# Alanlee0323/ISWM

Measured on AMD Instinct MI355X. Metric: training images/sec (513x513) DeepLabV3+-ResNet101, higher is better.
Workload: dtype f32; 1 GPU; deeplabv3plus_resnet101 output_stride=16, 513x513 synthetic tiles, 16 images/GPU (BASELINE.json configs[2]: global batch 128 over 8 GPUs), weighted CE [1,3], SGD-nesterov + cosine LR; fp32 tensors, conv products via six bf16 MFMAs on an exact 3-way operand split (bf16x6, fp32-level error); conv_math=bf16x6, global_batch=16, parallelism=dp1

## Files before the change

### include/iswm_hip.h

```cpp
#ifndef ISWM_HIP_H
#define ISWM_HIP_H

#include <stddef.h>
#include <stdint.h>

#ifdef __cplusplus
extern "C" {
#endif

typedef void* iswm_stream_t;

const char* iswm_last_error(void);
int iswm_version(void);

typedef struct {
    int N, H, W, Cin;
    int Ho, Wo, Cout;
    int KH, KW, stride, pad, dil;
    int ldx;
    int ldy;
} iswm_conv_desc;

int iswm_set_conv_math(int mode);
int iswm_get_conv_math(void);
// ... 73 lines not shown
int iswm_conv2d_wgrad_planes(const iswm_conv_desc* d, const void* xp, int64_t x_ps, const void* dyp, int64_t dy_ps, float* dw,
                             float* workspace, size_t workspace_bytes, iswm_stream_t stream);
int iswm_dwconv2d_fwd(const iswm_conv_desc* d, const float* x, const float* w, int Cw, const float* bias, float* y,
                      iswm_stream_t stream);
int iswm_dwconv2d_dgrad(const iswm_conv_desc* d, const float* dy, const float* w, int Cw, float* dx, int accumulate,
                        iswm_stream_t stream);
size_t iswm_dwconv2d_wgrad_workspace(const iswm_conv_desc* d);
int iswm_dwconv2d_wgrad(const iswm_conv_desc* d, const float* x, const float* dy, int Cw, float* dw, void* workspace,
                        size_t workspace_bytes, iswm_stream_t stream);
size_t iswm_conv2d_wgrad_workspace(const iswm_conv_desc* d);
int iswm_conv2d_wgrad(const iswm_conv_desc* d, const float* x, const float* dy, float* dw,
                      float* workspace, size_t workspace_bytes, iswm_stream_t stream);

int iswm_colstat_tiles(int64_t M);
int64_t iswm_colstat_tile_rows(int64_t M);
int iswm_colstat(const float* x, int64_t M, int C, int ld, float* partials, iswm_stream_t stream);
int iswm_bn_finalize(const float* partials, int tiles, int C, int64_t count, int64_t tile_rows,
                     const float* gamma, const float* beta, float* running_mean, float* running_var, float momentum,
                     float eps, float* scale, float* shift, float* save_mean, float* save_invstd,
                     iswm_stream_t stream);
int iswm_bn_eval_coeffs(int C, const float* gamma, const float* beta, const float* running_mean,
                        const float* running_var, float eps, float* scale, float* shift,
                        float* save_mean, float* save_invstd, iswm_stream_t stream);
int iswm_bn_apply(const float* y, int64_t M, int C, int ldy, const float* scale, const float* shift,
                  const float* mean, const float* residual, int ldr, int relu, float* out, int ldo,
                  iswm_stream_t stream);
size_t iswm_bn_bwd_workspace(int64_t M, int C);
int iswm_bn_backward(const float* dout, int ldd, const float* out, int ldo, const float* y, int ldy,
                     int64_t M, int C, const float* mean, const float* invstd, const float* gamma,
                     const float* mask_scale, const float* mask_shift,
                     int relu, int training, float* dgamma, float* dbeta, float* dy, int lddy,
                     float* dres, int lddres, void* workspace, size_t workspace_bytes,
                     iswm_stream_t stream);
int iswm_colsum_finalize(const float* partials, int tiles, int C, float* out, float* scratch,
                         iswm_stream_t stream);

int iswm_maxpool3x3s2_fwd(const float* x, int N, int H, int W, int C, float* y, uint8_t* idx, int Ho,
                          int Wo, iswm_stream_t stream);
int iswm_maxpool3x3s2_bwd(const float* dy, const uint8_t* idx, int N, int H, int W, int C, int Ho,
                          int Wo, float* dx, iswm_stream_t stream);
int iswm_gap_fwd(const float* x, int N, int HW, int C, int ldx, float* y, iswm_stream_t stream);
int iswm_gap_bwd(const float* dy, int N, int HW, int C, float* dx, int lddx, int accumulate,
                 iswm_stream_t stream);
int iswm_bcast_fwd(const float* v, int N, int HW, int C, float* y, int ldy, iswm_stream_t stream);
int iswm_bcast_bwd(const float* dy, int lddy, int N, int HW, int C, float* dv, iswm_stream_t stream);

int iswm_bilinear_fwd(const float* x, int N, int Hi, int Wi, int C, int ldx, float* y, int Ho, int Wo,
                      int ldy, iswm_stream_t stream);
int iswm_bilinear_bwd(const float* dy, int N, int Hi, int Wi, int C, int lddy, int Ho, int Wo, float* dx,
                      int lddx, iswm_stream_t stream);
int iswm_bilinear_nhwc_to_nchw_fwd(const float* x, int N, int Hi, int Wi, int C, int ldx, float* y,
                                   int Ho, int Wo, iswm_stream_t stream);
int iswm_bilinear_nhwc_to_nchw_bwd(const float* dy, int N, int Hi, int Wi, int C, int lddx, int Ho,
                                   int Wo, float* dx, iswm_stream_t stream);

int iswm_nchw_to_nhwc(const float* x, int N, int C, int HW, float* y, int Cp, iswm_stream_t stream);
int iswm_nhwc_to_nchw(const float* x, int N, int C, int HW, int ldx, float* y, iswm_stream_t stream);
int iswm_copy_channels(const float* src, int lds, float* dst, int ldd, int64_t M, int C,
                       iswm_stream_t stream);
int iswm_add_inplace(float* dst, const float* src, int64_t n, iswm_stream_t stream);
int iswm_scale_inplace(float* x, int64_t n, const float* scalar_dev, float host_mul, iswm_stream_t stream);
int iswm_bn_apply_classify(const float* y, int64_t M, int C, int ldy, const float* scale, const float* shift, const float* mean,
                           const float* wc4, const float* bias4, float* logits, int ldl, iswm_stream_t stream);
size_t iswm_bn_classify_bwd_workspace(int64_t M, int C);
int iswm_bn_backward_classify(const float* dlogit, int ldl, const float* wc4, const float* y, int ldy, int64_t M, int C,
                              const float* mean, const float* invstd, const float* gamma, const float* mask_scale,
// ... 118 lines not shown
```

### iswm_amd/_lib.py

```python
import ctypes
import os
from ctypes import POINTER, Structure, c_char_p, c_double, c_float, c_int, c_int64, c_size_t, c_uint64, c_void_p

HERE = os.path.dirname(os.path.abspath(__file__))
LIB_PATH = os.path.join(HERE, "libiswm_hip.so")


class ConvDesc(Structure):
    _fields_ = [(n, c_int) for n in ("N", "H", "W", "Cin", "Ho", "Wo", "Cout", "KH", "KW", "stride", "pad",
                                     "dil", "ldx", "ldy")]


class QConvDesc(Structure):
    _fields_ = [(n, c_int) for n in ("N", "H", "W", "Cin", "Ho", "Wo", "Cout", "KH", "KW", "stride", "pad",
                                     "dil", "ldx", "ldy", "ldr", "relu", "lo", "out_f32", "cstore")]


P = c_void_p
_SIGS = {
    "iswm_last_error": (c_char_p, []),
    "iswm_version": (c_int, []),
    "iswm_set_conv_math": (c_int, [c_int]),
    "iswm_get_conv_math": (c_int, []),
    "iswm_conv2d_kernel_name": (c_int, [POINTER(ConvDesc), c_int, c_char_p, c_int]),
# ... 20 lines not shown
    "iswm_maxpool3x3s2_fwd_pl": (c_int, [P, c_int, c_int, c_int, c_int, P, c_int64, P, c_int, c_int, P]),
    "iswm_gap_fwd_pl": (c_int, [P, c_int64, c_int, c_int, c_int, c_int, P, P]),
    "iswm_bcast_fwd_pl": (c_int, [P, c_int, c_int, c_int, P, c_int, c_int64, P]),
    "iswm_bilinear_fwd_pl": (c_int, [P, c_int, c_int, c_int, c_int, c_int, P, c_int64, c_int, c_int, c_int, P]),
    "iswm_conv2d_pl2_weight_bytes": (c_size_t, [POINTER(ConvDesc), c_int]),
    "iswm_conv2d_pl2_pack_weights": (c_int, [POINTER(ConvDesc), c_int, P, P, P]),
    "iswm_conv2d_pl2_tile_rows": (c_int, [POINTER(ConvDesc), c_int]),
    "iswm_conv2d_fwd_pl2": (c_int, [POINTER(ConvDesc), P, c_int64, P, P, P, P, P]),
    "iswm_conv2d_dgrad_pl2": (c_int, [POINTER(ConvDesc), P, c_int64, P, P, c_int, P]),
    "iswm_conv2d_dgrad_pl2_stat_tiles": (c_int, [POINTER(ConvDesc)]),
    "iswm_conv2d_dgrad_pl2_bn": (c_int, [POINTER(ConvDesc), P, c_int64, P, P, c_int, P, c_int, P, P, P, P, c_int, P, c_int, P,
                                         c_int, P]),
    "iswm_bn_backward_stats_pl": (c_int, [P, c_int, P, c_int, c_int64, P, c_int, c_int64, c_int, P, P, P, P, P, c_int, c_int, P, P,
                                          P, c_int, c_int64, P, c_int, P, c_int, P, c_size_t, P]),
    "iswm_aspp_plan_bytes": (c_size_t, [POINTER(ConvDesc), c_int, POINTER(c_int), POINTER(c_int), c_int]),
    "iswm_aspp_plan": (c_int, [POINTER(ConvDesc), c_int, POINTER(c_int), POINTER(c_int), c_int, P, c_int]),
    "iswm_aspp_fwd": (c_int, [POINTER(ConvDesc), c_int, POINTER(c_int), POINTER(c_int), P, P, c_int64, POINTER(c_void_p),
                              POINTER(c_void_p), POINTER(c_void_p), P]),
    "iswm_aspp_bwd": (c_int, [POINTER(ConvDesc), c_int, POINTER(c_int), POINTER(c_int), P, P, c_int64, c_int, POINTER(c_void_p), P,
                              c_int, P, c_int64, POINTER(c_void_p), P, c_size_t, P]),
    "iswm_conv2d_wgrad_planes_ok": (c_int, [POINTER(ConvDesc)]),
    "iswm_conv2d_wgrad_planes_workspace": (c_size_t, [POINTER(ConvDesc)]),
    "iswm_conv2d_wgrad_planes": (c_int, [POINTER(ConvDesc), P, c_int64, P, c_int64, P, P, c_size_t, P]),
    "iswm_conv2d_wgrad_workspace": (c_size_t, [POINTER(ConvDesc)]),
    "iswm_dwconv2d_fwd": (c_int, [POINTER(ConvDesc), P, P, c_int, P, P, P]),
    "iswm_dwconv2d_dgrad": (c_int, [POINTER(ConvDesc), P, P, c_int, P, c_int, P]),
    "iswm_dwconv2d_wgrad_workspace": (c_size_t, [POINTER(ConvDesc)]),
    "iswm_dwconv2d_wgrad": (c_int, [POINTER(ConvDesc), P, P, c_int, P, P, c_size_t, P]),
    "iswm_conv2d_wgrad": (c_int, [POINTER(ConvDesc), P, P, P, P, c_size_t, P]),
    "iswm_colstat_tiles": (c_int, [c_int64]),
    "iswm_colstat_tile_rows": (c_int64, [c_int64]),
    "iswm_colstat": (c_int, [P, c_int64, c_int, c_int, P, P]),
    "iswm_bn_finalize": (c_int, [P, c_int, c_int, c_int64, c_int64, P, P, P, P, c_float, c_float, P, P, P, P, P]),
    "iswm_bn_eval_coeffs": (c_int, [c_int, P, P, P, P, c_float, P, P, P, P, P]),
    "iswm_bn_apply": (c_int, [P, c_int64, c_int, c_int, P, P, P, P, c_int, c_int, P, c_int, P]),
    "iswm_bn_bwd_workspace": (c_size_t, [c_int64, c_int]),
    "iswm_bn_backward": (c_int, [P, c_int, P, c_int, P, c_int, c_int64, c_int, P, P, P, P, P, c_int, c_int, P, P, P, c_int,
                                 P, c_int, P, c_size_t, P]),
    "iswm_colsum_finalize": (c_int, [P, c_int, c_int, P, P, P]),
    "iswm_maxpool3x3s2_fwd": (c_int, [P, c_int, c_int, c_int, c_int, P, P, c_int, c_int, P]),
    "iswm_maxpool3x3s2_bwd": (c_int, [P, P, c_int, c_int, c_int, c_int, c_int, c_int, P, P]),
    "iswm_gap_fwd": (c_int, [P, c_int, c_int, c_int, c_int, P, P]),
    "iswm_gap_bwd": (c_int, [P, c_int, c_int, c_int, P, c_int, c_int, P]),
    "iswm_bcast_fwd": (c_int, [P, c_int, c_int, c_int, P, c_int, P]),
    "iswm_bcast_bwd": (c_int, [P, c_int, c_int, c_int, c_int, P, P]),
    "iswm_bilinear_fwd": (c_int, [P, c_int, c_int, c_int, c_int, c_int, P, c_int, c_int, c_int, P]),
    "iswm_bilinear_bwd": (c_int, [P, c_int, c_int, c_int, c_int, c_int, c_int, c_int, P, c_int, P]),
    "iswm_bilinear_nhwc_to_nchw_fwd": (c_int, [P, c_int, c_int, c_int, c_int, c_int, P, c_int, c_int, P]),
    "iswm_bilinear_nhwc_to_nchw_bwd": (c_int, [P, c_int, c_int, c_int, c_int, c_int, c_int, c_int, P, P]),
    "iswm_nchw_to_nhwc": (c_int, [P, c_int, c_int, c_int, P, c_int, P]),
    "iswm_nhwc_to_nchw": (c_int, [P, c_int, c_int, c_int, c_int, P, P]),
    "iswm_copy_channels": (c_int, [P, c_int, P, c_int, c_int64, c_int, P]),
    "iswm_add_inplace": (c_int, [P, P, c_int64, P]),
    "iswm_scale_inplace": (c_int, [P, c_int64, P, c_float, P]),
    "iswm_bn_apply_classify": (c_int, [P, c_int64, c_int, c_int, P, P, P, P, P, P, c_int, P]),
    "iswm_bn_classify_bwd_workspace": (c_size_t, [c_int64, c_int]),
    "iswm_bn_backward_classify": (c_int, [P, c_int, P, P, c_int, c_int64, c_int, P, P, P, P, P, c_int, P, P, P, P, c_int, c_int64,
                                          P, c_size_t, P]),
    "iswm_pad_weights": (c_int, [P, c_int, c_int, c_int, c_int, P, c_int, c_int, P, P]),
    "iswm_unpad_weights": (c_int, [P, c_int, c_int, c_int, c_int, c_int, c_int, P, P, P]),
    "iswm_fill_zero": (c_int, [P, c_size_t, P]),
    "iswm_zero_cols": (c_int, [P, c_int64, c_int64, c_int, c_int, c_int64, c_int, P]),
    "iswm_dropout_fwd": (c_int, [P, P, P, c_int64, c_float, c_uint64, c_uint64, P]),
    "iswm_dropout_bwd": (c_int, [P, P, P, c_int64, c_float, P]),
    "iswm_loss_blocks": (c_int, [c_int64]),
    "iswm_loss_fwd": (c_int, [P, P, c_int, c_int, c_int, c_int64, P, c_int, c_float, c_float, c_int, P, P, P]),
# ... 71 lines not shown
```

### iswm_amd/csrc/bn.hip

```cpp
#include <stdlib.h>

#include "rowmap.h"

namespace iswm {

__global__ __launch_bounds__(256) void k_colstat(const float* __restrict__ x, int64_t M, int C4, int ld,
                                                 int CQ, int RL, int tiles, int C, int64_t R,
                                                 float* __restrict__ partials) {
    __shared__ float red[256 * 4];
    __shared__ float mean_s[256 * 4];
    RowThread rt = row_thread(C4, CQ, RL);
    const int t = threadIdx.x;
    const int64_t r_begin = (int64_t)blockIdx.x * R;
    const int64_t r_end = min(M, r_begin + R);
    const float cnt = (float)(r_end - r_begin);
    const float* p = x + rt.c4 * 4;
    float4 s = make_float4(0, 0, 0, 0);
    if (rt.active)
        for (int64_t r = r_begin + rt.rl; r < r_end; r += RL) {
            float4 v = ld4(p + r * ld);
            s.x += v.x; s.y += v.y; s.z += v.z; s.w += v.w;
        }
    st4(&red[t * 4], s);
    __syncthreads();
// ... 350 lines not shown
    }
    for (int64_t r = rt.row0; r < M; r += rt.rstep) {
        float4 g = ld4(dout + r * ldd + c);
        float4 v = make_float4(0.f, 0.f, 0.f, 0.f);
        if (TRAIN || RELU == 2) v = ld4(y + r * ldy + c);
        if (RELU == 1) {
            float4 o = ld4x_hi(out, r * ldo + c, ops);
            g.x = o.x > 0.f ? g.x : 0.f; g.y = o.y > 0.f ? g.y : 0.f;
            g.z = o.z > 0.f ? g.z : 0.f; g.w = o.w > 0.f ? g.w : 0.f;
        } else if (RELU == 3) {
            float4 o = ld4x_hi(out, r * ldo + c, ops);
            g.x = (o.x > 0.f && o.x < 6.f) ? g.x : 0.f; g.y = (o.y > 0.f && o.y < 6.f) ? g.y : 0.f;
            g.z = (o.z > 0.f && o.z < 6.f) ? g.z : 0.f; g.w = (o.w > 0.f && o.w < 6.f) ? g.w : 0.f;
        } else if (RELU == 2) {
            g.x = (v.x - mu.x) * msc.x + msh.x > 0.f ? g.x : 0.f;
            g.y = (v.y - mu.y) * msc.y + msh.y > 0.f ? g.y : 0.f;
            g.z = (v.z - mu.z) * msc.z + msh.z > 0.f ? g.z : 0.f;
            g.w = (v.w - mu.w) * msc.w + msh.w > 0.f ? g.w : 0.f;
        }
        if (DRES) st4(dres + r * lddres + c, g);
        const double gd[4] = {g.x, g.y, g.z, g.w};
        float d[4];
        if (TRAIN) {
            const double vd[4] = {v.x, v.y, v.z, v.w};
#pragma unroll
            for (int k = 0; k < 4; ++k)
                d[k] = (float)(gi[k] * (gd[k] - k1[k] - (vd[k] - mud[k]) * isd[k] * k2[k]));
        } else {
#pragma unroll
            for (int k = 0; k < 4; ++k) d[k] = (float)(gi[k] * gd[k]);
        }
        st4x(dy, r * lddy + c, dyps, make_float4(d[0], d[1], d[2], d[3]));
    }
}

static int chk_rows(const char* what, int64_t M, int C, int ld) {
    ISWM_REQUIRE(M > 0 && C > 0 && C % 4 == 0 && ld % 4 == 0 && ld >= C, "%s: bad shape M=%lld C=%d ld=%d", what,
                 (long long)M, C, ld);
    return 0;
}

}

using namespace iswm;

extern "C" int iswm_colstat_tiles(int64_t M) {
    int64_t t = (M + 31) / 32;
    if (t > 1024) t = 1024;
    if (t < 1) t = 1;
    return (int)t;
}

extern "C" int64_t iswm_colstat_tile_rows(int64_t M) {
    const int64_t tiles = iswm_colstat_tiles(M);
    return (M + tiles - 1) / tiles;
}

extern "C" int iswm_colstat(const float* x, int64_t M, int C, int ld, float* partials, iswm_stream_t stream) {
    if (int e = chk_rows("colstat", M, C, ld)) return e;
    ISWM_REQUIRE(x && partials && aligned16(x) && aligned16(partials), "colstat: bad pointer");
    const int64_t R = iswm_colstat_tile_rows(M);
    const int tiles = (int)((M + R - 1) / R);
    RowPlan p = plan_rows(M, C, tiles);
    hipLaunchKernelGGL(k_colstat, dim3(p.rowblocks, p.colblocks), dim3(256), 0, (hipStream_t)stream, x, M, p.C4,
                       ld, p.CQ, p.RL, tiles, C, R, partials);
    return check_launch("colstat");
// ... 56 lines not shown
    hipStream_t s = (hipStream_t)stream;
    if (out_ps != 0 && C % 8 == 0 && ldy % 8 == 0 && ldo % 8 == 0 && aligned16(out) && (out_ps < 0 || out_ps % 8 == 0) &&
        (!residual || (ldr % 8 == 0 && aligned16(residual) && (res_ps <= 0 || res_ps % 8 == 0)))) {
        RowPlan p = plan_rows(M, C / 2);
        dim3 grid(p.rowblocks, p.colblocks), blk(256);
#define LAUNCH8(R, S) \
    hipLaunchKernelGGL((k_bn_apply8<R, S>), grid, blk, 0, s, y, M, p.C4, ldy, scale, shift, mean, residual, ldr, rps, out, \
                       ldo, ops, p.CQ, p.RL)
        ISWM_REQUIRE(relu == 0 || relu == 1 || relu == 6, "bn_apply: relu must be 0 (none), 1 (ReLU) or 6 (ReLU6)");
        if (relu == 6 && residual) LAUNCH8(2, true);
        else if (relu == 6) LAUNCH8(2, false);
        else if (relu && residual) LAUNCH8(1, true);
        else if (relu) LAUNCH8(1, false);
        else if (residual) LAUNCH8(0, true);
        else LAUNCH8(0, false);
#undef LAUNCH8
        return check_launch("bn_apply8");
    }
    RowPlan p = plan_rows(M, C);
    dim3 grid(p.rowblocks, p.colblocks), blk(256);
#define LAUNCH(R, S) \
    hipLaunchKernelGGL((k_bn_apply<R, S>), grid, blk, 0, s, y, M, p.C4, ldy, scale, shift, mean, residual, ldr, rps, out, \
                       ldo, ops, \
                       p.CQ, p.RL)
    ISWM_REQUIRE(relu == 0 || relu == 1 || relu == 6, "bn_apply: relu must be 0 (none), 1 (ReLU) or 6 (ReLU6)");
    if (relu == 6 && residual) LAUNCH(2, true);
    else if (relu == 6) LAUNCH(2, false);
    else if (relu && residual) LAUNCH(1, true);
    else if (relu) LAUNCH(1, false);
    else if (residual) LAUNCH(0, true);
    else LAUNCH(0, false);
#undef LAUNCH
    return check_launch("bn_apply");
}

extern "C" size_t iswm_bn_bwd_workspace(int64_t M, int C) {
    return ((size_t)2 * iswm_colstat_tiles(M) * C + (size_t)2 * C) * sizeof(double);
}

extern "C" int iswm_bn_backward(const float* dout, int ldd, const float* out, int ldo, const float* y, int ldy,
                                int64_t M, int C, const float* mean, const float* invstd, const float* gamma,
                                const float* mask_scale, const float* mask_shift,
                                int relu, int training, float* dgamma, float* dbeta, float* dy, int lddy,
                                float* dres, int lddres, void* workspace, size_t workspace_bytes,
                                iswm_stream_t stream) {
    return iswm_bn_backward_pl(dout, ldd, out, ldo, 0, y, ldy, M, C, mean, invstd, gamma, mask_scale, mask_shift, relu,
                               training, dgamma, dbeta, dy, lddy, 0, dres, lddres, workspace, workspace_bytes, stream);
}

static int bn_backward_impl(const float* dout, int ldd, const void* out, int ldo, int64_t out_ps, const float* y,
                            int ldy, int64_t M, int C, const float* mean, const float* invstd, const float* gamma,
                            const float* mask_scale, const float* mask_shift, int relu, int training,
                            float* dgamma, float* dbeta, void* dy, int lddy, int64_t dy_ps, float* dres,
                            int lddres, void* workspace, size_t workspace_bytes, const double* ready_partials,
                            int ready_tiles, iswm_stream_t stream) {
    if (int e = chk_rows("bn_backward", M, C, ldy)) return e;
    if (int e = chk_ps("bn_backward(dy)", dy, M, lddy, dy_ps)) return e;
    if (out) if (int e = chk_ps("bn_backward(out)", out, M, ldo, out_ps)) return e;
    const int64_t ops = out_ps, dyps = dy_ps;
    ISWM_REQUIRE(relu == 0 || relu == 1 || relu == 6, "bn_backward: relu must be 0 (none), 1 (ReLU) or 6 (ReLU6)");
    const bool relu6 = relu == 6;
    const bool masky = relu == 1 && !dres && mask_scale && mask_shift;
    ISWM_REQUIRE(dout && y && mean && invstd && dgamma && dbeta && dy && workspace && (!relu || out || masky),
                 "bn_backward: null pointer");
    ISWM_REQUIRE(ldd % 4 == 0 && ldd >= C && lddy % 4 == 0 && lddy >= C && (!relu || (ldo % 4 == 0 && ldo >= C)) &&
                     (!dres || (lddres % 4 == 0 && lddres >= C)),
                 "bn_backward: bad pitch");
    ISWM_REQUIRE(workspace_bytes >= iswm_bn_bwd_workspace(M, C) && aligned16(workspace),
                 "bn_backward: workspace too small");
    const int tiles = ready_partials ? ready_tiles : iswm_colstat_tiles(M);
    const double* partials = ready_partials ? ready_partials : (const double*)workspace;
    double* sums = (double*)workspace + (size_t)2 * iswm_colstat_tiles(M) * C;
    hipStream_t s = (hipStream_t)stream;
    if (!ready_partials) {
        double* partials = (double*)workspace;
        RowPlan p = plan_rows(M, C, tiles);
        dim3 grid(p.rowblocks, p.colblocks), blk(256);
#define RLAUNCH(R, D)                                                                                           \
    hipLaunchKernelGGL((k_bn_bwd_reduce<R, D>), grid, blk, 0, s, dout, ldd, out, ldo, ops, y, ldy, M, p.C4, C, mean, invstd, \
                       mask_scale, mask_shift, p.CQ, p.RL, tiles, partials)
        const bool dbl = M <= 8192;
        if (relu6 && dbl) RLAUNCH(3, true);
        else if (relu6) RLAUNCH(3, false);
        else if (masky && dbl) RLAUNCH(2, true);
        else if (masky) RLAUNCH(2, false);
        else if (relu && dbl) RLAUNCH(1, true);
        else if (relu) RLAUNCH(1, false);
        else if (dbl) RLAUNCH(0, true);
        else RLAUNCH(0, false);
#undef RLAUNCH
        if (int e = check_launch("bn_bwd_reduce")) return e;
    }
    if (tiles > 32)
        hipLaunchKernelGGL((k_bn_bwd_finalize<double, 4>), dim3((C + 3) / 4), dim3(256), 0, s, partials, tiles, C,
                           dgamma, dbeta, sums);
    else
        hipLaunchKernelGGL((k_bn_bwd_finalize<double, 16>), dim3((C + 15) / 16), dim3(256), 0, s, partials, tiles, C,
                           dgamma, dbeta, sums);
    if (int e = check_launch("bn_bwd_finalize")) return e;
    const double inv = 1.0 / (double)M;
    RowPlan p = plan_rows(M, C);
    dim3 grid(p.rowblocks, p.colblocks), blk(256);
#define LAUNCH(R, T, D)                                                                                          \
    hipLaunchKernelGGL((k_bn_bwd_apply<R, T, D>), grid, blk, 0, s, dout, ldd, out, ldo, ops, y, ldy, M, p.C4, C, mean,    \
                       invstd, gamma, mask_scale, mask_shift, sums, inv, dy, lddy, dyps, dres, lddres, p.CQ, p.RL)
    const int key = (relu ? 4 : 0) | (training ? 2 : 0) | (dres ? 1 : 0);
    if (relu6) {
        if (training && dres) LAUNCH(3, true, true);
        else if (training) LAUNCH(3, true, false);
        else if (dres) LAUNCH(3, false, true);
        else LAUNCH(3, false, false);
    } else if (masky) {
        if (training) LAUNCH(2, true, false);
        else LAUNCH(2, false, false);
    } else switch (key) {
        case 0: LAUNCH(0, false, false); break;
        case 1: LAUNCH(0, false, true); break;
        case 2: LAUNCH(0, true, false); break;
        case 3: LAUNCH(0, true, true); break;
        case 4: LAUNCH(1, false, false); break;
        case 5: LAUNCH(1, false, true); break;
        case 6: LAUNCH(1, true, false); break;
        default: LAUNCH(1, true, true); break;
    }
#undef LAUNCH
// ... 34 lines not shown
```

### iswm_amd/network/_hip.py

```python

import torch
import torch.nn as nn

from .. import ops


MASK_RECORDER = None
POOL_RECORDER = None
CALIB_RECORDER = None


def pad4(c):
    return (c + 3) // 4 * 4


def pad_cin(c):
    if c % 32 == 0 or c < 128:
        return pad4(c)
    return (c + 31) // 32 * 32


def dense_flat(t):
    if t.dim() == 4 and not t.is_contiguous():
        v = t.permute(0, 2, 3, 1)
# ... 250 lines not shown
    sep = None
    if isinstance(conv, SeparableBase):
        sep, conv = conv, conv.body[1]
        x = sep.body[0].fwd(x, save)
    training = bn.training
    if bn.momentum is None or not bn.track_running_stats or not bn.affine:
        raise NotImplementedError("HIP BatchNorm2d supports affine=True, momentum!=None, running stats")
    if isinstance(conv, DepthwiseConv2d):
        g = conv.geometry(x)
        y = conv.fwd(x, save)
        partials, tiles = None, (0, 0)
        if training:
            partials, nt, tr = ops.colstat(y)
            tiles = (nt, tr)
        return _cba_finish(conv, bn, relu, x, y, g, partials, tiles, training, save, residual, out, sep, True, out_fmt)
    g = conv.geometry(x)
    if conv.bias is None:
        y, partials, tiles = ops.conv2d_fwd(x, conv.ohwi(), g, want_stats=training, wpk=conv.packed(0), wpk2=conv.packed2(0))
    else:
        y, _, _ = ops.conv2d_fwd(x, conv.ohwi(), g, bias=conv.bias_p())
        partials, tiles = None, (0, 0)
        if training:
            partials, nt, tr = ops.colstat(y)
            tiles = (nt, tr)
    return _cba_finish(conv, bn, relu, x, y, g, partials, tiles, training, save, residual, out, sep, False, out_fmt)


def _cba_finish(conv, bn, relu, x, y, g, partials, tiles, training, save, residual, out, sep, dw, out_fmt=None):
    if training:
        count = y.shape[0] * y.shape[1] * y.shape[2]
        if count <= 1:
            raise ValueError("Expected more than 1 value per channel when training, got input size %s" %
                             (tuple(y.shape),))
        coef = ops.bn_finalize(partials, tiles[0], count, tiles[1], bn.weight, bn.bias, bn.running_mean, bn.running_var,
                               bn.momentum, bn.eps)
        if not getattr(bn, "_iswm_nbt_fused", False):
            bn.num_batches_tracked.add_(1)
    else:
        coef = ops.bn_eval_coeffs(bn.weight, bn.bias, bn.running_mean, bn.running_var, bn.eps)
    if out_fmt is None:
        want_planes = ops.planes_on() and y.shape[3] % 64 == 0
    else:
        want_planes = out_fmt == "planes" and ops.planes_on() and y.shape[3] % 64 == 0
    o = ops.bn_apply(y, coef, relu, residual, out, planes=want_planes)
    if MASK_RECORDER is not None and relu:
        of = ops.as_f32(o)
        MASK_RECORDER[bn] = (of > 0) & (of < 6) if relu == 6 and relu is not True else (of > 0)
    if CALIB_RECORDER is not None:
        CALIB_RECORDER.record(conv, o)
    ctx = None
    if save:
        ctx = dict(x=x, y=y, out=o, coef=coef, g=g, relu=relu, training=training, res=residual is not None, sep=sep, dw=dw)
    return o, ctx


_BN3_FUSE = True


def _bn_stats_request(up):
    if up is None or not ops.planes_on() or up.get("bn_stats") is not None:
        return None
    if ops._relu_code(up["relu"]) not in (0, 1):
        return None
    if up.get("res"):
        if not (_BN3_FUSE and ops._relu_code(up["relu"]) == 1 and ops.is_planes(up["out"]) and up["training"]):
            return None
        return ops.BnStats(up["y"], up["coef"], up["relu"], mask=up["out"])
    return ops.BnStats(up["y"], up["coef"], up["relu"])


def cba_bwd_bn(conv, bn, ctx, dout, sink, dy_out=None, need_dx=True):
    y, o = ctx["y"], ctx["out"]
    sep = ctx.get("sep")
    if sep is not None:
        conv = sep.body[1]
    gw, gb = bn.weight, bn.bias
    dgamma = sink.target(gw) if gw.requires_grad else torch.empty_like(gw)
# ... 271 lines not shown
```

### iswm_amd/ops.py

```python
import ctypes
import functools

import torch

from . import _lib
from ._lib import ConvDesc, call

BN_EPS = 1e-5


def _stream():
    return ctypes.c_void_p(torch.cuda.current_stream().cuda_stream)


def _p(t):
    return ctypes.c_void_p(t.data_ptr()) if t is not None else None


def geom(t, dtype=torch.float32):
    if isinstance(t, Planes):
        raise ValueError("this operation takes an fp32 NHWC tensor, not Planes (use .f32())")
    if t.dim() != 4 or t.dtype != dtype or not t.is_cuda:
        raise ValueError("expected a 4-D fp32 CUDA NHWC tensor, got %s %s %s" % (tuple(t.shape), t.dtype, t.device))
    n, h, w, c = t.shape
# ... 600 lines not shown
    coef = torch.empty((4, c), dtype=torch.float32, device=partials.device)
    call("iswm_bn_finalize", _p(partials), tiles, c, count, tile_rows, _p(gamma), _p(beta), _p(running_mean),
         _p(running_var), float(momentum), float(eps), _p(coef[0]), _p(coef[1]), _p(coef[2]), _p(coef[3]), _stream())
    return coef


def bn_eval_coeffs(gamma, beta, running_mean, running_var, eps=BN_EPS):
    c = running_mean.numel()
    coef = torch.empty((4, c), dtype=torch.float32, device=running_mean.device)
    call("iswm_bn_eval_coeffs", c, _p(gamma), _p(beta), _p(running_mean), _p(running_var), float(eps), _p(coef[0]),
         _p(coef[1]), _p(coef[2]), _p(coef[3]), _stream())
    return coef


def _relu_code(relu):
    return 6 if (relu == 6 and relu is not True) else int(bool(relu))


def bn_apply(y, coef, relu, residual=None, out=None, planes=False):
    m, c, ldy = rows(y)
    if out is None:
        out = new_planes(*y.shape, y.device) if planes else torch.empty(y.shape, dtype=torch.float32, device=y.device)
    po, mo, co, ldo, pso = xrows(out)
    assert (mo, co) == (m, c)
    pr, ldr, psr = None, 0, 0
    if residual is not None:
        pr, mr, cr, ldr, psr = xrows(residual)
        assert (mr, cr) == (m, c)
    call("iswm_bn_apply_pl", _p(y), m, c, ldy, _p(coef[0]), _p(coef[1]), _p(coef[2]), _p(pr), ldr, psr, _relu_code(relu),
         _p(po), ldo, pso, _stream())
    return out


def bn_backward(dout, out, y, coef, gamma, relu, training, dgamma, dbeta, want_dres=False, dy=None, dy_planes=False,
                stats=None):
    m, c, ldy = rows(y)
    _, _, ldd = rows(dout)
    po, ldo, pso = None, 0, 0
    if out is not None:
        po, _, _, ldo, pso = xrows(out)
    need = _lib.load().iswm_bn_bwd_workspace(m, c)
    ws = torch.empty((need // 8,), dtype=torch.float64, device=y.device)
    if dy is None:
        dy = new_planes(*y.shape, y.device) if dy_planes else torch.empty(y.shape, dtype=torch.float32, device=y.device)
    pdy, _, _, lddy, psdy = xrows(dy)
    dres = torch.empty(y.shape, dtype=torch.float32, device=y.device) if want_dres else None
    masky = _relu_code(relu) == 1 and not want_dres
    if stats is not None and stats.partials is not None:
        call("iswm_bn_backward_stats_pl", _p(dout), ldd, _p(po), ldo, pso, _p(y), ldy, m, c, _p(coef[2]), _p(coef[3]), _p(gamma),
             _p(coef[0]) if masky else None, _p(coef[1]) if masky else None,
             _relu_code(relu), int(bool(training)), _p(dgamma), _p(dbeta), _p(pdy), lddy, psdy, _p(dres),
             rows(dres)[2] if dres is not None else 0, _p(stats.partials), stats.tiles, _p(ws), need, _stream())
        return dy, dres
    call("iswm_bn_backward_pl", _p(dout), ldd, _p(po), ldo, pso, _p(y), ldy, m, c, _p(coef[2]), _p(coef[3]), _p(gamma),
         _p(coef[0]) if masky else None, _p(coef[1]) if masky else None,
         _relu_code(relu), int(bool(training)), _p(dgamma), _p(dbeta), _p(pdy), lddy, psdy, _p(dres),
         rows(dres)[2] if dres is not None else 0, _p(ws), need, _stream())
    return dy, dres


def bn_apply_classify(y, coef, wc4, bias4):
    m, c, ldy = rows(y)
    out = torch.empty(tuple(y.shape[:3]) + (4,), dtype=torch.float32, device=y.device)
    call("iswm_bn_apply_classify", _p(y), m, c, ldy, _p(coef[0]), _p(coef[1]), _p(coef[2]), _p(wc4), _p(bias4), _p(out), 4, _stream())
    return out

# ... 465 lines not shown
```

Measured before the change: 268.1 images/sec.

## Fold BN statistic finalization into the apply and backward-apply kernels

Adds fused kernels that reduce the per-tile BN partial sums to mean/variance (or dgamma/dbeta) inside each block and then apply the normalization or backward input-gradient in the same launch. This removes a separate finalize launch and its global round-trip for the coefficients, in both forward and backward training paths. Each block redundantly re-reduces the partials for its channel group, adding duplicated reduction work and shared-memory use. The fused path applies only when tiles is between 33 and 128 and C is a multiple of 32; otherwise it falls back to the old two-step path.

```diff
diff --git a/include/iswm_hip.h b/include/iswm_hip.h
--- a/include/iswm_hip.h
+++ b/include/iswm_hip.h
@@ -129,6 +129,13 @@
                      int relu, int training, float* dgamma, float* dbeta, float* dy, int lddy,
                      float* dres, int lddres, void* workspace, size_t workspace_bytes,
                      iswm_stream_t stream);
+int iswm_bn_finalize_apply_pl(const float* partials, int tiles, int C, int64_t count, int64_t tile_rows,
+                              const float* gamma, const float* beta, float* running_mean, float* running_var,
+                              float momentum, float eps, float* scale, float* shift, float* save_mean,
+                              float* save_invstd, const float* y, int64_t M, int ldy, const void* residual, int ldr,
+                              int64_t res_ps, int relu, void* out, int ldo, int64_t out_ps, iswm_stream_t stream);
+int iswm_bn_set_fold(int on);
+int iswm_bn_fold_applies(int tiles, int C);
 int iswm_colsum_finalize(const float* partials, int tiles, int C, float* out, float* scratch,
                          iswm_stream_t stream);
 
diff --git a/iswm_amd/_lib.py b/iswm_amd/_lib.py
--- a/iswm_amd/_lib.py
+++ b/iswm_amd/_lib.py
@@ -76,6 +76,10 @@
     "iswm_colstat_tile_rows": (c_int64, [c_int64]),
     "iswm_colstat": (c_int, [P, c_int64, c_int, c_int, P, P]),
     "iswm_bn_finalize": (c_int, [P, c_int, c_int, c_int64, c_int64, P, P, P, P, c_float, c_float, P, P, P, P, P]),
+    "iswm_bn_finalize_apply_pl": (c_int, [P, c_int, c_int, c_int64, c_int64, P, P, P, P, c_float, c_float, P, P, P, P,
+                                          P, c_int64, c_int, P, c_int, c_int64, c_int, P, c_int, c_int64, P]),
+    "iswm_bn_set_fold": (c_int, [c_int]),
+    "iswm_bn_fold_applies": (c_int, [c_int, c_int]),
     "iswm_bn_eval_coeffs": (c_int, [c_int, P, P, P, P, c_float, P, P, P, P, P]),
     "iswm_bn_apply": (c_int, [P, c_int64, c_int, c_int, P, P, P, P, c_int, c_int, P, c_int, P]),
     "iswm_bn_bwd_workspace": (c_size_t, [c_int64, c_int]),
diff --git a/iswm_amd/csrc/bn.hip b/iswm_amd/csrc/bn.hip
--- a/iswm_amd/csrc/bn.hip
+++ b/iswm_amd/csrc/bn.hip
@@ -406,6 +406,283 @@
         }
         st4x(dy, r * lddy + c, dyps, make_float4(d[0], d[1], d[2], d[3]));
     }
+}
+
+constexpr int FOLD_G = 32;
+constexpr int FOLD_TL = 64;
+constexpr int FOLD_LPT = FOLD_TL * FOLD_G / 256;
+constexpr int FOLD_MAX_TILES = 2 * FOLD_TL;
+
+template <int RELU, bool RES, bool W8>
+__global__ __launch_bounds__(256) void k_bn_fin_apply(const float* __restrict__ partials, int tiles, int C, double count,
+                                                      double R, const float* __restrict__ gamma,
+                                                      const float* __restrict__ beta, float* running_mean,
+                                                      float* running_var, float momentum, float eps, float* scale,
+                                                      float* shift, float* save_mean, float* save_invstd,
+                                                      const float* __restrict__ y, int64_t M, int ldy,
+                                                      const void* __restrict__ res, int ldr, int64_t rps,
+                                                      void* __restrict__ out, int ldo, int64_t ops) {
+    constexpr int NU = W8 ? 2 : 1;
+    constexpr int TPR = FOLD_G / (4 * NU);
+    constexpr int RLN = 256 / TPR;
+    __shared__ double red[FOLD_TL][FOLD_G];
+    __shared__ double mean_s[FOLD_G];
+    __shared__ __align__(16) float coef_s[3][FOLD_G];
+    __shared__ double nt_s[FOLD_MAX_TILES];
+    const int t = threadIdx.x;
+    const int c0 = blockIdx.y * FOLD_G;
+    const int cq = (t % TPR) * 4 * NU;
+    const int c = c0 + cq;
+    int64_t r = (int64_t)blockIdx.x * RLN + t / TPR;
+    const int64_t rstep = (int64_t)gridDim.x * RLN;
+    const float4 z4 = make_float4(0.f, 0.f, 0.f, 0.f);
+    float4 v[2][NU], q[2][NU];
+    auto load = [&](int64_t r0) {
+#pragma unroll
+        for (int u = 0; u < 2; ++u) {
+            const int64_t rr = r0 + u * rstep;
+#pragma unroll
+            for (int n = 0; n < NU; ++n) v[u][n] = q[u][n] = z4;
+            if (rr < M) {
+#pragma unroll
+                for (int n = 0; n < NU; ++n) v[u][n] = ld4(y + rr * ldy + c + 4 * n);
+                if (RES) {
+                    if constexpr (W8) ld8x(res, rr * ldr + c, rps, q[u][0], q[u][1]);
+                    else q[u][0] = ld4x(res, rr * ldr + c, rps);
+                }
+            }
+        }
+    };
+    load(r);
+
+    const int cl = t % FOLD_G, j = t / FOLD_G;
+    const int pc = c0 + cl;
+    float sv[FOLD_LPT][2], qv[FOLD_LPT][2];
+    const float* ps = partials + c0;
+    const float* pq = ps + (size_t)tiles * C;
+#pragma unroll
+    for (int i = 0; i < FOLD_LPT; ++i)
+#pragma unroll
+        for (int h = 0; h < 2; ++h) {
+            const int k = j + FOLD_LPT * i + FOLD_TL * h;
+            const unsigned off = (unsigned)(min(k, tiles - 1) * C + cl);
+            sv[i][h] = ps[off];
+            qv[i][h] = pq[off];
+        }
+#pragma unroll
+    for (int i = 0; i < FOLD_LPT; ++i)
+#pragma unroll
+        for (int h = 0; h < 2; ++h)
+            if (j + FOLD_LPT * i + FOLD_TL * h >= tiles) sv[i][h] = qv[i][h] = 0.f;
+    if (t < tiles) nt_s[t] = R > 0.0 ? fmin(R, count - (double)t * R) : (double)partials[(size_t)2 * tiles * C + t];
+#pragma unroll
+    for (int i = 0; i < FOLD_LPT; ++i) {
+        double s = 0.0;
+        s += (double)sv[i][0];
+        s += (double)sv[i][1];
+        red[j + FOLD_LPT * i][cl] = s;
+    }
+    __syncthreads();
+    if (t < FOLD_G) {
+        double s = red[0][cl];
+#pragma unroll 9
+        for (int k = 1; k < FOLD_TL; ++k) s += red[k][cl];
+        mean_s[cl] = s / count;
+    }
+    __syncthreads();
+    const double mean = mean_s[cl];
+#pragma unroll
+    for (int i = 0; i < FOLD_LPT; ++i) {
+        double m2 = 0.0;
+#pragma unroll
+        for (int h = 0; h < 2; ++h) {
+            const int k = j + FOLD_LPT * i + FOLD_TL * h;
+            if (k < tiles) {
+                const double nt = nt_s[k];
+                const double d = (double)sv[i][h] / nt - mean;
+                m2 += (double)qv[i][h] + nt * d * d;
+            }
+        }
+        red[j + FOLD_LPT * i][cl] = m2;
+        __builtin_amdgcn_sched_barrier(0);
+    }
+    __syncthreads();
+    if (t < FOLD_G) {
+        double m2 = red[0][cl];
+#pragma unroll 9
+        for (int k = 1; k < FOLD_TL; ++k) m2 += red[k][cl];
+        double var = m2 / count;
+        if (var < 0.0) var = 0.0;
+        float invstd = (float)(1.0 / sqrt(var + (double)eps));
+        float g = gamma ? gamma[pc] : 1.f, b = beta ? beta[pc] : 0.f;
+        float sc = g * invstd;
+        coef_s[0][cl] = sc;
+        coef_s[1][cl] = b;
+        coef_s[2][cl] = (float)mean;
+        if (blockIdx.x == 0) {
+            scale[pc] = sc;
+            shift[pc] = b;
+            save_mean[pc] = (float)mean;
+            save_invstd[pc] = invstd;
+            if (running_mean) {
+                double unbiased = count > 1.0 ? var * count / (count - 1.0) : var;
+                running_mean[pc] = __fadd_rn(__fmul_rn(1.f - momentum, running_mean[pc]), __fmul_rn(momentum, (float)mean));
+                running_var[pc] = __fmaf_rn(momentum, (float)unbiased, __fmul_rn(1.f - momentum, running_var[pc]));
+            }
+        }
+    }
+    __syncthreads();
+    float4 sc[NU], sh[NU], mu[NU];
+#pragma unroll
+    for (int n = 0; n < NU; ++n) {
+        sc[n] = ld4(&coef_s[0][cq + 4 * n]);
+        sh[n] = ld4(&coef_s[1][cq + 4 * n]);
+        mu[n] = ld4(&coef_s[2][cq + 4 * n]);
+    }
+    auto one = [&](int64_t rr, const float4* vv, const float4* qq) {
+        float4 o[NU];
+#pragma unroll
+        for (int n = 0; n < NU; ++n) {
+            o[n].x = (vv[n].x - mu[n].x) * sc[n].x + sh[n].x; o[n].y = (vv[n].y - mu[n].y) * sc[n].y + sh[n].y;
+            o[n].z = (vv[n].z - mu[n].z) * sc[n].z + sh[n].z; o[n].w = (vv[n].w - mu[n].w) * sc[n].w + sh[n].w;
+            if (RES) {
+                o[n].x += qq[n].x; o[n].y += qq[n].y; o[n].z += qq[n].z; o[n].w += qq[n].w;
+            }
+            if (RELU) {
+                o[n].x = fmaxf(o[n].x, 0.f); o[n].y = fmaxf(o[n].y, 0.f); o[n].z = fmaxf(o[n].z, 0.f); o[n].w = fmaxf(o[n].w, 0.f);
+            }
+            if (RELU == 2) {
+                o[n].x = fminf(o[n].x, 6.f); o[n].y = fminf(o[n].y, 6.f); o[n].z = fminf(o[n].z, 6.f); o[n].w = fminf(o[n].w, 6.f);
+            }
+        }
+        if constexpr (W8) st8x(out, rr * ldo + c, ops, o[0], o[1]);
+        else st4x(out, rr * ldo + c, ops, o[0]);
+    };
+    while (r < M) {
+        one(r, v[0], q[0]);
+        if (r + rstep < M) one(r + rstep, v[1], q[1]);
+        r += 2 * rstep;
+        if (r < M) load(r);
+    }
+}
+
+template <int RELU, bool DRES>
+__global__ __launch_bounds__(256, 5) void k_bn_bwd_fin_apply(const float* __restrict__ dout, int ldd,
+                                                          const void* __restrict__ out, int ldo, int64_t ops,
+                                                          const float* __restrict__ y, int ldy, int64_t M, int C,
+                                                          const float* __restrict__ mean, const float* __restrict__ invstd,
+                                                          const float* __restrict__ gamma, const float* __restrict__ mscale,
+                                                          const float* __restrict__ mshift,
+                                                          const double* __restrict__ partials, int tiles, double inv_count,
+                                                          float* dgamma, float* dbeta, void* __restrict__ dy, int lddy,
+                                                          int64_t dyps, float* __restrict__ dres, int lddres) {
+    constexpr int TPR = FOLD_G / 4, RLN = 256 / TPR;
+    __shared__ double red[FOLD_TL][FOLD_G];
+    __shared__ double sum_s[2][FOLD_G];
+    const int t = threadIdx.x;
+    const int c0 = blockIdx.y * FOLD_G;
+    const int cq = (t % TPR) * 4;
+    const int c = c0 + cq;
+    int64_t r = (int64_t)blockIdx.x * RLN + t / TPR;
+    const int64_t rstep = (int64_t)gridDim.x * RLN;
+    const float4 z4 = make_float4(0.f, 0.f, 0.f, 0.f);
+    float4 g = z4, v = z4, o = z4;
+    auto load_o = [&](int64_t rr) {
+        if (RELU == 1 || RELU == 3) o = ld4x_hi(out, rr * ldo + c, ops);
+    };
+    auto load = [&](int64_t rr) {
+        g = ld4(dout + rr * ldd + c);
+        v = ld4(y + rr * ldy + c);
+    };
+    if (r < M) load(r);
+
+    const int cl = t % FOLD_G, j = t / FOLD_G;
+    const int pc = c0 + cl;
+#pragma unroll
+    for (int w = 0; w < 2; ++w) {
+        const double* pw = partials + (size_t)w * tiles * C + c0;
+        double a[FOLD_LPT][2];
+#pragma unroll
+        for (int i = 0; i < FOLD_LPT; ++i)
+#pragma unroll
+            for (int h = 0; h < 2; ++h) {
+                const int k = j + FOLD_LPT * i + FOLD_TL * h;
+                a[i][h] = pw[(unsigned)(min(k, tiles - 1) * C + cl)];
+            }
+        if (w) __syncthreads();
+#pragma unroll
+        for (int i = 0; i < FOLD_LPT; ++i) {
+            const int tl = j + FOLD_LPT * i;
+            double s = 0.0;
+            if (tl + FOLD_TL < tiles) s += a[i][0] + a[i][1];
+            else if (tl < tiles) s += a[i][0];
+            red[tl][cl] = s;
+        }
+        __syncthreads();
+        if (t < FOLD_G) {
+            double s = red[0][cl];
+    #pragma unroll 9
+        for (int k = 1; k < FOLD_TL; ++k) s += red[k][cl];
+            sum_s[w][cl] = s;
+            if (blockIdx.x == 0) (w ? dgamma : dbeta)[pc] = (float)s;
+        }
+    }
+    __syncthreads();
+    const float4 mu = ld4(mean + c), is = ld4(invstd + c);
+    const float4 ga = gamma ? ld4(gamma + c) : make_float4(1.f, 1.f, 1.f, 1.f);
+    const double mud[4] = {mu.x, mu.y, mu.z, mu.w}, isd[4] = {is.x, is.y, is.z, is.w};
+    const double gi[4] = {(double)ga.x * is.x, (double)ga.y * is.y, (double)ga.z * is.z, (double)ga.w * is.w};
+    float4 msc = z4, msh = z4;
+    if (RELU == 2) {
+        msc = ld4(mscale + c);
+        msh = ld4(mshift + c);
+    }
+    double k1[4], k2[4];
+#pragma unroll
+    for (int k = 0; k < 4; ++k) {
+        k1[k] = sum_s[0][cq + k] * inv_count;
+        k2[k] = sum_s[1][cq + k] * inv_count;
+    }
+    if (r < M) load_o(r);
+    while (r < M) {
+        if (RELU == 1) {
+            g.x = o.x > 0.f ? g.x : 0.f; g.y = o.y > 0.f ? g.y : 0.f;
+            g.z = o.z > 0.f ? g.z : 0.f; g.w = o.w > 0.f ? g.w : 0.f;
+        } else if (RELU == 3) {
+            g.x = (o.x > 0.f && o.x < 6.f) ? g.x : 0.f; g.y = (o.y > 0.f && o.y < 6.f) ? g.y : 0.f;
+            g.z = (o.z > 0.f && o.z < 6.f) ? g.z : 0.f; g.w = (o.w > 0.f && o.w < 6.f) ? g.w : 0.f;
+        } else if (RELU == 2) {
+            g.x = (v.x - mu.x) * msc.x + msh.x > 0.f ? g.x : 0.f;
+            g.y = (v.y - mu.y) * msc.y + msh.y > 0.f ? g.y : 0.f;
+            g.z = (v.z - mu.z) * msc.z + msh.z > 0.f ? g.z : 0.f;
+            g.w = (v.w - mu.w) * msc.w + msh.w > 0.f ? g.w : 0.f;
+        }
+        if (DRES) st4(dres + r * lddres + c, g);
+        const double gd[4] = {g.x, g.y, g.z, g.w}, vd[4] = {v.x, v.y, v.z, v.w};
+        float d[4];
+#pragma unroll
+        for (int k = 0; k < 4; ++k) d[k] = (float)(gi[k] * (gd[k] - k1[k] - (vd[k] - mud[k]) * isd[k] * k2[k]));
+        st4x(dy, r * lddy + c, dyps, make_float4(d[0], d[1], d[2], d[3]));
+        r += rstep;
+        if (r < M) {
+            load(r);
+            load_o(r);
+        }
+    }
+}
+
+static int g_bn_fold = 1;
+
+static bool bn_fold_ok(int tiles, int C) {
+    return g_bn_fold && tiles > 32 && tiles <= FOLD_MAX_TILES && C % FOLD_G == 0;
+}
+
+static int fold_rowblocks(int64_t M, int row_lanes, int colgroups) {
+    int64_t rb = (M + (int64_t)row_lanes * 4 - 1) / ((int64_t)row_lanes * 4);
+    int64_t cap = 8192 / colgroups;
+    if (cap < 1) cap = 1;
+    if (rb > cap) rb = cap;
+    return (int)rb;
 }
 
 static int chk_rows(const char* what, int64_t M, int C, int ld) {
@@ -528,6 +805,59 @@
     else LAUNCH(0, false);
 #undef LAUNCH
     return check_launch("bn_apply");
+}
+
+extern "C" int iswm_bn_finalize_apply_pl(const float* partials, int tiles, int C, int64_t count, int64_t tile_rows,
+                                         const float* gamma, const float* beta, float* running_mean, float* running_var,
+                                         float momentum, float eps, float* scale, float* shift, float* save_mean,
+                                         float* save_invstd, const float* y, int64_t M, int ldy, const void* residual, int ldr,
+                                         int64_t res_ps, int relu, void* out, int ldo, int64_t out_ps, iswm_stream_t stream) {
+    ISWM_REQUIRE(count == M, "bn_finalize_apply: count %lld != rows %lld", (long long)count, (long long)M);
+    if (!bn_fold_ok(tiles, C)) {
+        if (int e = iswm_bn_finalize(partials, tiles, C, count, tile_rows, gamma, beta, running_mean, running_var, momentum, eps,
+                                     scale, shift, save_mean, save_invstd, stream))
+            return e;
+        return iswm_bn_apply_pl(y, M, C, ldy, scale, shift, save_mean, residual, ldr, res_ps, relu, out, ldo, out_ps, stream);
+    }
+    ISWM_REQUIRE(partials && scale && shift && save_mean && save_invstd && count > 0 && tile_rows >= 0 &&
+                     (tile_rows == 0 || (int64_t)tiles == (count + tile_rows - 1) / tile_rows),
+                 "bn_finalize_apply: bad argument (tiles %d, count %lld, tile_rows %lld)", tiles, (long long)count,
+                 (long long)tile_rows);
+    if (int e = chk_rows("bn_finalize_apply", M, C, ldy)) return e;
+    ISWM_REQUIRE(y && out && ldo % 4 == 0 && ldo >= C && aligned16(y), "bn_finalize_apply: bad argument");
+    ISWM_REQUIRE(!residual || (ldr % 4 == 0 && ldr >= C), "bn_finalize_apply: bad residual pitch");
+    if (int e = chk_ps("bn_finalize_apply(out)", out, M, ldo, out_ps)) return e;
+    if (residual) if (int e = chk_ps("bn_finalize_apply(residual)", residual, M, ldr, res_ps)) return e;
+    ISWM_REQUIRE(relu == 0 || relu == 1 || relu == 6, "bn_finalize_apply: relu must be 0 (none), 1 (ReLU) or 6 (ReLU6)");
+    const int64_t rps = res_ps, ops = out_ps;
+    const double cnt = (double)count, R = (double)tile_rows;
+    hipStream_t s = (hipStream_t)stream;
+    const bool w8 = out_ps != 0 && ldy % 8 == 0 && ldo % 8 == 0 && aligned16(out) && (out_ps < 0 || out_ps % 8 == 0) &&
+                    (!residual || (ldr % 8 == 0 && aligned16(residual) && (res_ps <= 0 || res_ps % 8 == 0)));
+    const int groups = C / FOLD_G;
+    dim3 grid(fold_rowblocks(M, w8 ? 64 : 32, groups), groups), blk(256);
+#define FLAUNCH(R_, S_, W_)                                                                                                  \
+    hipLaunchKernelGGL((k_bn_fin_apply<R_, S_, W_>), grid, blk, 0, s, partials, tiles, C, cnt, R, gamma, beta, running_mean, \
+                       running_var, momentum, eps, scale, shift, save_mean, save_invstd, y, M, ldy, residual, ldr, rps, out, \
+                       ldo, ops)
+#define FLAUNCH_W(R_, S_) do { if (w8) FLAUNCH(R_, S_, true); else FLAUNCH(R_, S_, false); } while (0)
+    if (relu == 6 && residual) FLAUNCH_W(2, true);
+    else if (relu == 6) FLAUNCH_W(2, false);
+    else if (relu && residual) FLAUNCH_W(1, true);
+    else if (relu) FLAUNCH_W(1, false);
+    else if (residual) FLAUNCH_W(0, true);
+    else FLAUNCH_W(0, false);
+#undef FLAUNCH_W
+#undef FLAUNCH
+    return check_launch("bn_finalize_apply");
+}
+
+extern "C" int iswm_bn_fold_applies(int tiles, int C) { return bn_fold_ok(tiles, C) ? 1 : 0; }
+
+extern "C" int iswm_bn_set_fold(int on) {
+    const int was = g_bn_fold;
+    g_bn_fold = on ? 1 : 0;
+    return was;
 }
 
 extern "C" size_t iswm_bn_bwd_workspace(int64_t M, int C) {
@@ -587,6 +917,23 @@
 #undef RLAUNCH
         if (int e = check_launch("bn_bwd_reduce")) return e;
     }
+    if (training && bn_fold_ok(tiles, C)) {
+        const int groups = C / FOLD_G;
+        dim3 grid(fold_rowblocks(M, 256 / (FOLD_G / 4), groups), groups), blk(256);
+        const double inv = 1.0 / (double)M;
+#define FLAUNCH(R, D)                                                                                                      \
+    hipLaunchKernelGGL((k_bn_bwd_fin_apply<R, D>), grid, blk, 0, s, dout, ldd, out, ldo, ops, y, ldy, M, C, mean, invstd, gamma, \
+                       mask_scale, mask_shift, partials, tiles, inv, dgamma, dbeta, dy, lddy, dyps, dres, lddres)
+        if (relu6 && dres) FLAUNCH(3, true);
+        else if (relu6) FLAUNCH(3, false);
+        else if (masky) FLAUNCH(2, false);
+        else if (relu && dres) FLAUNCH(1, true);
+        else if (relu) FLAUNCH(1, false);
+        else if (dres) FLAUNCH(0, true);
+        else FLAUNCH(0, false);
+#undef FLAUNCH
+        return check_launch("bn_bwd_fin_apply");
+    }
     if (tiles > 32)
         hipLaunchKernelGGL((k_bn_bwd_finalize<double, 4>), dim3((C + 3) / 4), dim3(256), 0, s, partials, tiles, C,
                            dgamma, dbeta, sums);
diff --git a/iswm_amd/network/_hip.py b/iswm_amd/network/_hip.py
--- a/iswm_amd/network/_hip.py
+++ b/iswm_amd/network/_hip.py
@@ -306,17 +306,18 @@
         if count <= 1:
             raise ValueError("Expected more than 1 value per channel when training, got input size %s" %
                              (tuple(y.shape),))
-        coef = ops.bn_finalize(partials, tiles[0], count, tiles[1], bn.weight, bn.bias, bn.running_mean, bn.running_var,
-                               bn.momentum, bn.eps)
         if not getattr(bn, "_iswm_nbt_fused", False):
             bn.num_batches_tracked.add_(1)
-    else:
-        coef = ops.bn_eval_coeffs(bn.weight, bn.bias, bn.running_mean, bn.running_var, bn.eps)
     if out_fmt is None:
         want_planes = ops.planes_on() and y.shape[3] % 64 == 0
     else:
         want_planes = out_fmt == "planes" and ops.planes_on() and y.shape[3] % 64 == 0
-    o = ops.bn_apply(y, coef, relu, residual, out, planes=want_planes)
+    if training:
+        o, coef = ops.bn_finalize_apply(y, partials, tiles[0], tiles[1], bn.weight, bn.bias, bn.running_mean, bn.running_var,
+                                        bn.momentum, bn.eps, relu, residual, out, planes=want_planes)
+    else:
+        coef = ops.bn_eval_coeffs(bn.weight, bn.bias, bn.running_mean, bn.running_var, bn.eps)
+        o = ops.bn_apply(y, coef, relu, residual, out, planes=want_planes)
     if MASK_RECORDER is not None and relu:
         of = ops.as_f32(o)
         MASK_RECORDER[bn] = (of > 0) & (of < 6) if relu == 6 and relu is not True else (of > 0)
diff --git a/iswm_amd/ops.py b/iswm_amd/ops.py
--- a/iswm_amd/ops.py
+++ b/iswm_amd/ops.py
@@ -656,6 +656,38 @@
     return out
 
 
+BN_FOLD = True
+
+
+def set_bn_fold(on):
+    global BN_FOLD
+    was, BN_FOLD = BN_FOLD, bool(on)
+    _lib.load().iswm_bn_set_fold(int(BN_FOLD))
+    return was
+
+
+def bn_finalize_apply(y, partials, tiles, tile_rows, gamma, beta, running_mean, running_var, momentum, eps, relu, residual=None,
+                      out=None, planes=False):
+    if not BN_FOLD:
+        m = rows(y)[0]
+        coef = bn_finalize(partials, tiles, m, tile_rows, gamma, beta, running_mean, running_var, momentum, eps)
+        return bn_apply(y, coef, relu, residual, out, planes), coef
+    m, c, ldy = rows(y)
+    coef = torch.empty((4, c), dtype=torch.float32, device=y.device)
+    if out is None:
+        out = new_planes(*y.shape, y.device) if planes else torch.empty(y.shape, dtype=torch.float32, device=y.device)
+    po, mo, co, ldo, pso = xrows(out)
+    assert (mo, co) == (m, c)
+    pr, ldr, psr = None, 0, 0
+    if residual is not None:
+        pr, mr, cr, ldr, psr = xrows(residual)
+        assert (mr, cr) == (m, c)
+    call("iswm_bn_finalize_apply_pl", _p(partials), tiles, c, m, tile_rows, _p(gamma), _p(beta), _p(running_mean),
+         _p(running_var), float(momentum), float(eps), _p(coef[0]), _p(coef[1]), _p(coef[2]), _p(coef[3]), _p(y), m, ldy, _p(pr),
+         ldr, psr, _relu_code(relu), _p(po), ldo, pso, _stream())
+    return out, coef
+
+
 def bn_backward(dout, out, y, coef, gamma, relu, training, dgamma, dbeta, want_dres=False, dy=None, dy_planes=False,
                 stats=None):
     m, c, ldy = rows(y)
```

New measurement: 263.0 images/sec. 0.981x the previous value.
